# KAdamek/SMFFT

Measured on AMD Instinct MI355X. Metric: batched_ffts_per_sec_N1024_c2c_fwd_4GiB_external, higher is better.
Workload: dtype f32

## Files before the change

include/smfft/smfft_dif.hpp:

```cpp
#pragma once
#include "smfft_device_functions.hpp"

namespace smfft {

template <int N>
struct DifPlan {
    static constexpr int kBits = ilog2c(N);
    static constexpr bool kOdd = (kBits & 1) != 0;
    static constexpr int kQuads = kBits / 2;
    static constexpr int kPasses = kQuads + (kOdd ? 1 : 0);
    static constexpr bool radix2(int j) { return kOdd && j == 0; }
    __host__ __device__ static constexpr int span(int j) { return 1 << (2 * (kQuads - 1 - (j - (kOdd ? 1 : 0)))); }
    __host__ __device__ static constexpr int element(int j, int t, int m) {
        return radix2(j) ? t + m * (N / 4) : ((t / span(j)) * 4 * span(j)) + (t % span(j)) + m * span(j);
    }
    static constexpr bool crosses_waves(int j) { return N > 256 && (radix2(j) || span(j) >= 256); }
    __host__ __device__ static constexpr int twiddle_index(int j, int t) {
        return radix2(j) ? (t * (4096 / N)) & 4095 : span(j) == 1 ? -1 : ((t % span(j)) * (4096 / (4 * span(j)))) & 4095;
    }
    __host__ __device__ static constexpr int twiddle_row_entry(int j, int t) {
        return radix2(j) ? QuarterTwiddleRows<N>::row_start(QuarterTwiddleRows<N>::kPasses) + t
                         : QuarterTwiddleRows<N>::row_start(ilog2c(span(j)) / 2) + t % span(j);
    }
};

template <int DIR>
__device__ __forceinline__ float2 dif_mul_mi(float2 v) { return DIR ? make_float2(-v.y, v.x) : make_float2(v.y, -v.x); }

template <int DIR>
__device__ __forceinline__ void dif_quad_butterfly(float2 (&e)[4], float2 w2, bool trivial) {
    const float2 s0 = cadd(e[0], e[2]), d0 = csub(e[0], e[2]), s1 = cadd(e[1], e[3]);
    const float2 d1 = dif_mul_mi<DIR>(csub(e[1], e[3]));
    e[0] = cadd(s0, s1);
    if (trivial) {
        e[1] = csub(s0, s1), e[2] = cadd(d0, d1), e[3] = csub(d0, d1);
    } else {
        const float2 w1 = make_float2(w2.x * w2.x - w2.y * w2.y, 2.f * w2.x * w2.y);
        e[1] = cmul(csub(s0, s1), w1), e[2] = cmul(cadd(d0, d1), w2), e[3] = cmul(csub(d0, d1), cmul(w1, w2));
    }
}

template <int N, int DIR, int BLOCK_THREADS, bool IN_REGS, bool OUT_REGS>
__device__ __forceinline__ void dif_ladder(float2 (&x)[4], float2* s, int t, int region_offset) {
    using D = DifPlan<N>;
    constexpr bool kMulti = BLOCK_THREADS > 64;
    float2 w[D::kPasses];
#pragma unroll
    for (int j = 0; j < D::kPasses; ++j) {
        w[j] = make_float2(1.f, 0.f);
        if (D::radix2(j) || D::span(j) > 1) {
            const TwiddleValue tv = quarter_twiddle_rows<N>.w[D::twiddle_row_entry(j, t)];
            w[j] = make_float2(tv.x, DIR ? -tv.y : tv.y);
        }
    }
    float2 e[4];
#pragma unroll
    for (int m = 0; m < 4; ++m) e[m] = IN_REGS ? x[m] : s[region_offset + t + m * (N / 4)];
    if constexpr (!IN_REGS) fft_sync<kMulti>();
#pragma unroll
    for (int j = 0; j < D::kPasses; ++j) {
        if (j > 0) {
#pragma unroll
            for (int m = 0; m < 4; ++m) e[m] = s[quarter_swizzle(region_offset + D::element(j, t, m))];
        }
        if (D::radix2(j)) {
            const float2 a0 = cadd(e[0], e[2]), a1 = cadd(e[1], e[3]);
            const float2 b0 = cmul(csub(e[0], e[2]), w[j]), b1 = cmul(csub(e[1], e[3]), w[j]);
            e[0] = a0, e[1] = a1, e[2] = b0, e[3] = dif_mul_mi<DIR>(b1);
        } else {
            dif_quad_butterfly<DIR>(e, w[j], D::span(j) == 1);
        }
        if (j + 1 < D::kPasses) {
#pragma unroll
            for (int m = 0; m < 4; ++m) s[quarter_swizzle(region_offset + D::element(j, t, m))] = e[m];
            if (D::crosses_waves(j) && kMulti) fft_sync<true>();
            else fft_sync<false>();
        }
    }
    fft_sync<false>();
    if constexpr (OUT_REGS) {
#pragma unroll
        for (int m = 0; m < 4; ++m) x[m] = e[m];
    } else {
#pragma unroll
        for (int m = 0; m < 4; ++m) s[region_offset + 4 * t + m] = e[m];
    }
}

}

template <class const_params>
__device__ void do_SMFFT_CT_DIF(float2* s_input) {
    static_assert(const_params::fft_reorder == 0, "the DIF transform is the transpose of a no-reorder (FFT_<N>_*_noreorder) class");
    constexpr int N = const_params::fft_size;
    constexpr int kBlock = const_params::fft_length / 4;
    const int f = threadIdx.x / (N / 4), t = threadIdx.x % (N / 4);
    float2 x[4];
    smfft::dif_ladder<N, const_params::fft_direction, kBlock, false, false>(x, s_input, t, f * N);
}

template <class const_params>
__device__ void do_SMFFT_CT_DIF_registers(float2 (&x)[4], float2* s_scratch) {
    static_assert(const_params::fft_reorder == 0, "the DIF transform is the transpose of a no-reorder (FFT_<N>_*_noreorder) class");
    constexpr int N = const_params::fft_size;
    static_assert(N >= 256 && const_params::fft_length == N, "one transform per block of N / 4 threads");
    smfft::dif_ladder<N, const_params::fft_direction, N / 4, true, true>(x, s_scratch, threadIdx.x, 0);
}
```

Measured before the change: 395.7 million.

## Run last four DIF passes within a wave using lane swaps and one LDS exchange

Result: no change. 398.4 million, median of 3 (+0.7%).

```diff
diff --git a/include/smfft/smfft_dif.hpp b/include/smfft/smfft_dif.hpp
--- a/include/smfft/smfft_dif.hpp
+++ b/include/smfft/smfft_dif.hpp
@@ -40,10 +40,47 @@
     }
 }
 
+#ifndef SMFFT_DIF_EXCHANGE
+#define SMFFT_DIF_EXCHANGE -1
+#endif
+constexpr bool dif_exchange_through_block(int n) { return n >= 512 && (SMFFT_DIF_EXCHANGE < 0 ? true : SMFFT_DIF_EXCHANGE != 0); }
+
+template <int N, int DIR>
+struct DifLanes {
+    static constexpr bool kBlockExchange = dif_exchange_through_block(N);
+    __host__ __device__ static constexpr int element(int L, int lane, int m) { return (lane / L) * 4 * L + lane % L + m * L; }
+    using X = QuarterLanes<256, DIR, 0>;
+    __host__ __device__ static constexpr int exchange_store(int lane, int j) { return X::exchange_image((lane & 15) + 64 * (lane >> 4)) ^ X::exchange_image(16 * j); }
+    __host__ __device__ static constexpr int exchange_load(int lane, int j) { return X::exchange_image((lane & 3) + 16 * (lane >> 2)) ^ (4 * j); }
+    __device__ static __forceinline__ void run(float2 (&e)[4], float2 w64, float2 w16, float2 w4, float2* block, int lane, bool loads_precede) {
+        dif_quad_butterfly<DIR>(e, w64, false);
+        slots_swap<0, 4, true>(e);
+        slots_swap<1, 5, true>(e);
+        dif_quad_butterfly<DIR>(e, w16, false);
+        if constexpr (kBlockExchange) {
+            if (loads_precede) fft_sync<false>();
+#pragma unroll
+            for (int j = 0; j < 4; ++j) block[exchange_store(lane, j)] = e[j];
+            fft_sync<false>();
+#pragma unroll
+            for (int j = 0; j < 4; ++j) e[j] = block[exchange_load(lane, j)];
+        } else {
+            slots_swap<0, 2, true>(e);
+            slots_swap<1, 3, true>(e);
+        }
+        dif_quad_butterfly<DIR>(e, w4, false);
+        slots_swap<0, 0, true>(e);
+        slots_swap<1, 1, true>(e);
+        dif_quad_butterfly<DIR>(e, make_float2(1.f, 0.f), true);
+    }
+};
+
 template <int N, int DIR, int BLOCK_THREADS, bool IN_REGS, bool OUT_REGS>
 __device__ __forceinline__ void dif_ladder(float2 (&x)[4], float2* s, int t, int region_offset) {
     using D = DifPlan<N>;
     constexpr bool kMulti = BLOCK_THREADS > 64;
+    constexpr bool kLanesTail = N >= 256;
+    constexpr int kImagePasses = kLanesTail ? D::kPasses - 4 : D::kPasses;
     float2 w[D::kPasses];
 #pragma unroll
     for (int j = 0; j < D::kPasses; ++j) {
@@ -56,9 +93,9 @@
     float2 e[4];
 #pragma unroll
     for (int m = 0; m < 4; ++m) e[m] = IN_REGS ? x[m] : s[region_offset + t + m * (N / 4)];
-    if constexpr (!IN_REGS) fft_sync<kMulti>();
+    if constexpr (!IN_REGS && (!kLanesTail || N > 256)) fft_sync<kMulti>();
 #pragma unroll
-    for (int j = 0; j < D::kPasses; ++j) {
+    for (int j = 0; j < kImagePasses; ++j) {
         if (j > 0) {
 #pragma unroll
             for (int m = 0; m < 4; ++m) e[m] = s[quarter_swizzle(region_offset + D::element(j, t, m))];
@@ -76,6 +113,15 @@
             if (D::crosses_waves(j) && kMulti) fft_sync<true>();
             else fft_sync<false>();
         }
+    }
+    if constexpr (kLanesTail) {
+        constexpr int j64 = D::kPasses - 4;
+        static_assert(D::span(j64) == 64 && !D::crosses_waves(j64) && (j64 == 0 || D::crosses_waves(j64 - 1)), "the tail starts where the waves part");
+        if constexpr (j64 > 0) {
+#pragma unroll
+            for (int m = 0; m < 4; ++m) e[m] = s[quarter_swizzle(region_offset + D::element(j64, t, m))];
+        }
+        DifLanes<N, DIR>::run(e, w[j64], w[j64 + 1], w[j64 + 2], s + region_offset + 256 * (t >> 6), t & 63, true);
     }
     fft_sync<false>();
     if constexpr (OUT_REGS) {
```
